# vectorch-ai/ScaleLLM

Hardware: AMD Instinct MI355X
Metric: decode tokens/s (Llama-3-8B-shaped step, bs=256, seq=4k; paged-attention HBM roofline + int4-GEMM TFLOP/s alongside) (higher is better)
Workload: dtype bf16 (int4 weights, fp32 accumulate)

## Files before the change

### include/slm_hip.h

```cpp
#ifndef SLM_HIP_H_
#define SLM_HIP_H_

#include <stddef.h>
#include <stdint.h>

#ifdef __cplusplus
extern "C" {
#endif

#define SLM_API __attribute__((visibility("default")))

typedef enum slm_status {
  SLM_OK = 0,
  SLM_ERR_INVALID_ARG = -1,
  SLM_ERR_UNSUPPORTED = -2,
  SLM_ERR_WORKSPACE = -3,
  SLM_ERR_LAUNCH = -4,
  SLM_ERR_ALIGNMENT = -5
} slm_status;

typedef enum slm_dtype {
  SLM_F16 = 0,
  SLM_BF16 = 1,
  SLM_F32 = 2
// ... 98 lines not shown
  const int32_t* perm;
  const void* bias;
  void* c;
  int64_t M, K, N;
  int64_t lda, ldc;
  int64_t group_size;
  int32_t dtype;
  int32_t flags;
  void* workspace;
  size_t workspace_bytes;
} slm_w4_gemm_args;

#define SLM_W4_DEFER_REDUCE 1
#define SLM_W4_SILU_MUL 2
#define SLM_W4_SHARES_CHIP 4

SLM_API size_t slm_w4a16_gemm_workspace_bytes(const slm_w4_gemm_args* a);
SLM_API int32_t slm_w4a16_gemm_deferred_splits(const slm_w4_gemm_args* a);
typedef enum slm_w4_kernel {
  SLM_W4_KERNEL_GEMV = 0,
  SLM_W4_KERNEL_KS = 1,
  SLM_W4_KERNEL_SMALL = 2,
  SLM_W4_KERNEL_GENERAL = 3,
  SLM_W4_KERNEL_M128 = 4,
  SLM_W4_KERNEL_WS = 5,
  SLM_W4_KERNEL_XL = 6,
  SLM_W4_KERNEL_XL_SK = 7
} slm_w4_kernel;
typedef struct slm_w4_plan_info {
  int32_t kernel;
  int32_t row_tiles;
  int32_t n_mblocks, n_nblocks, split_k, chunks_per_split;
  int32_t variant[4];
  uint64_t lds_bytes;
  uint64_t part_bytes, aperm_bytes;
} slm_w4_plan_info;
SLM_API int slm_w4a16_gemm_plan(const slm_w4_gemm_args* a, slm_w4_plan_info* out);
SLM_API int slm_w4a16_gemm(const slm_w4_gemm_args* a, void* stream);

typedef struct slm_w4_norm_prologue {
  const void* x;
  const float* partials;
// ... 479 lines not shown
```

### scalellm_amd/_lib.py

```python
from __future__ import annotations

import ctypes as C
import os

_HERE = os.path.dirname(os.path.abspath(__file__))
LIB_PATH = os.path.join(_HERE, "csrc", "libslm_hip.so")

SLM_F16, SLM_BF16 = 0, 1
SLM_F32 = 2
SLM_SAMPLE_MAX_TOP = 20
SLM_REJECTION_MAX_K = 16
SLM_W4_GPTQ, SLM_W4_AWQ = 0, 1
SLM_W8_GPTQ, SLM_W8_AWQ = 2, 3
SLM_W4_PAIRED = 0x10


class SlmError(RuntimeError):
    pass


class AttnArgs(C.Structure):
    _fields_ = [
        ("out", C.c_void_p), ("query", C.c_void_p), ("key_cache", C.c_void_p),
        ("value_cache", C.c_void_p),
# ... 13 lines not shown

class W4GemmArgs(C.Structure):
    _fields_ = [
        ("a", C.c_void_p), ("wq", C.c_void_p), ("sz", C.c_void_p), ("perm", C.c_void_p),
        ("bias", C.c_void_p), ("c", C.c_void_p),
        ("M", C.c_int64), ("K", C.c_int64), ("N", C.c_int64),
        ("lda", C.c_int64), ("ldc", C.c_int64), ("group_size", C.c_int64),
        ("dtype", C.c_int32), ("flags", C.c_int32),
        ("workspace", C.c_void_p), ("workspace_bytes", C.c_size_t),
    ]


SLM_W4_DEFER_REDUCE = 1
SLM_W4_SILU_MUL = 2
SLM_W4_SHARES_CHIP = 4

W4_KERNELS = ("GEMV", "KS", "SMALL", "GENERAL", "M128", "WS", "XL", "XL_SK")


class W4PlanInfo(C.Structure):
    _fields_ = [
        ("kernel", C.c_int32), ("row_tiles", C.c_int32), ("n_mblocks", C.c_int32),
        ("n_nblocks", C.c_int32), ("split_k", C.c_int32), ("chunks_per_split", C.c_int32),
        ("variant", C.c_int32 * 4),
        ("lds_bytes", C.c_uint64), ("part_bytes", C.c_uint64), ("aperm_bytes", C.c_uint64),
    ]

    @property
    def kernel_name(self) -> str:
        return W4_KERNELS[self.kernel]


# ... 354 lines not shown
```

### scalellm_amd/cpp_host.py

```python
from __future__ import annotations

import importlib.util
import os

_shim = None


def load_shim():
    global _shim
    if _shim is None:
        from .build_shim import build
        path = build()
        spec = importlib.util.spec_from_file_location("_slm_shim", path)
        mod = importlib.util.module_from_spec(spec)
        spec.loader.exec_module(mod)
        _shim = mod
    return _shim


def cpp_params(params):
    shim = load_shim()
    q = shim.InputParameters()
    q.num_sequences = int(params.q_cu_seq_lens.numel() - 1)
    q.q_cu_seq_lens, q.kv_cu_seq_lens = params.q_cu_seq_lens, params.kv_cu_seq_lens
# ... 7 lines not shown
    shim = load_shim()
    q = shim.SamplingParameters()
    names = ["temperatures", "top_p", "top_k", "do_sample", "seeds"]
    if sp.unique_token_ids is not None:
        names += ["frequency_penalties", "presence_penalties", "repetition_penalties", "unique_token_ids",
                  "unique_token_counts", "unique_token_ids_lens"]
    for name in names:
        t = getattr(sp, name)
        if t is not None:
            setattr(q, name, t)
    q.logprobs, q.max_top_logprobs = bool(sp.logprobs), int(sp.max_top_logprobs)
    return q


def from_decode_step(step, block_size: int, max_tokens: int, fused: bool = True, lanes: int = -1,
                     lanes_chain: bool = True, rank: int = 0, world_size: int = 1, kv_step=None):
    from .decode import hf_state_dict
    shim = load_shim()
    s = step.shape
    if getattr(step, "dense", False):
        raise ValueError("the C++ host step is built for int4 checkpoints: it has no unquantised form")
    qa = step.layers[0]["qkv"].quant_args
    if qa.bits != 4 or qa.desc_act:
        raise ValueError("the C++ host step is built for 4-bit, non-act-order checkpoints")
    m = shim.LlamaForCausalLMHip(hidden=s.hidden, n_heads=s.n_heads, n_kv_heads=s.n_kv_heads, head_dim=s.head_dim,
                                 intermediate=s.intermediate, n_layers=s.n_layers, vocab=s.vocab,
                                 max_position=s.max_position, rope_theta=s.rope_theta, rms_eps=s.rms_eps,
                                 quant_method=qa.quant_method, bits=4, group_size=qa.group_size, desc_act=False,
                                 max_tokens=max_tokens, fused=fused, decode_lanes=lanes, lanes_chain=lanes_chain,
                                 device_index=step.device.index or 0, rank=rank, world_size=world_size)
    m.load_state_dict(hf_state_dict(step))
    m.verify_loaded_weights()
    m.set_kv_caches([(L["kv"].key_cache, L["kv"].value_cache) for L in (kv_step or step).layers], block_size)
    m.set_cos_sin_cache(step.attn.handler.cos_sin)
    m.reserve(max_tokens)
    return m
```

### scalellm_amd/csrc/capi.hip

```cpp
#include <atomic>
#include <mutex>
#include <stdlib.h>
#include <string.h>

#include "common.h"
#include "tuning.h"

namespace slm {

namespace {
const char* const kTuneNames[TUNE_COUNT] = {
    "SLM_ATTN_NW",          "SLM_ATTN_SPLITS",      "SLM_ATTN_HGW",     "SLM_ATTN_TILE",
    "SLM_ATTN_TILE_SPLITS", "SLM_ATTN_TILE_PF",     "SLM_ATTN_U",       "SLM_ATTN_NT",
    "SLM_ATTN_TILE_DECODE", "SLM_ATTN_BAL",         "SLM_ATTN_W",       "SLM_ATTN_PRIO",
    "SLM_W4_GEMV",          "SLM_W4_GEMV_KS",   "SLM_W4_SMALL",
    "SLM_W4_MT",            "SLM_W4_MT_WIDE",       "SLM_W4_NTW",           "SLM_W4_PC",        "SLM_W4_SPLITK",
    "SLM_W4_POST",
    "SLM_W4_KS",            "SLM_W4_KS_CW",         "SLM_W4_KS_NW",     "SLM_W4_KS_TPW",
    "SLM_W4_KS_MT2",
    "SLM_W4_M128",          "SLM_W4_M128_WD",       "SLM_W4_M128_SPLITS",   "SLM_W4_M128_KW",   "SLM_W4_SPLIT_TARGET",
    "SLM_W4_M128_CT",       "SLM_ATTN_TILE_KV2",    "SLM_W4_XL_MODEL",      "SLM_W4_M128_ADMA",
    "SLM_W4_XL_SK",
    "SLM_LINEAR_SPLITK",    "SLM_LINEAR_RT",        "SLM_LINEAR_NW",
};
std::atomic<int32_t> g_tune[TUNE_COUNT];
std::once_flag g_tune_once;

void tune_init() {
  for (int k = 0; k < TUNE_COUNT; ++k) {
    const char* v = getenv(kTuneNames[k]);
    g_tune[k].store((v && *v) ? (int32_t)atoi(v) : TUNE_UNSET, std::memory_order_relaxed);
  }
}
int tune_index(const char* name) {
  if (!name) return -1;
  for (int k = 0; k < TUNE_COUNT; ++k)
    if (strcmp(name, kTuneNames[k]) == 0) return k;
  return -1;
// ... 146 lines not shown
```

### scalellm_amd/csrc/shim/slm_llama_hip.cpp

```cpp
#include "slm_llama_hip.h"

#include <ATen/hip/HIPEvent.h>
#include <ATen/hip/impl/HIPGuardImplMasqueradingAsCUDA.h>
#include <ATen/hip/impl/HIPStreamMasqueradingAsCUDA.h>
#include <c10/hip/HIPGraphsC10Utils.h>

#include <cmath>

#include "slm_hip.h"
#include "slm_rejection_sampler_hip.h"

namespace slm {
namespace {

using Stream = c10::hip::HIPStreamMasqueradingAsCUDA;

int dt(const torch::Tensor& t) { return t.scalar_type() == torch::kBFloat16 ? SLM_BF16 : SLM_F16; }
void* cur(const torch::Tensor& t) {
  return c10::hip::getCurrentHIPStreamMasqueradingAsCUDA(t.device().index()).stream();
}
void ok(int rc, const char* what) {
  TORCH_CHECK(rc == SLM_OK, what, " failed: ", slm_status_string(rc), " (", rc, ")",
              rc == SLM_ERR_LAUNCH ? slm_last_hip_error() : "");
}
// ... 370 lines not shown
void LlamaForCausalLMHip::run_two_lanes(Lane& l0, Lane& l1, std::vector<KVCache>& kv) {
  const auto dev = options_.device().index();
  const Stream main = c10::hip::getCurrentHIPStreamMasqueradingAsCUDA(dev);
  if (!side_stream_.has_value()) {
    TORCH_CHECK(!capturing(), "LlamaForCausalLMHip: call reserve() before capturing a two-lane step");
    side_stream_ = c10::hip::getStreamFromPoolMasqueradingAsCUDA(false, dev);
  }
  const Stream side = *side_stream_;
  std::vector<std::unique_ptr<at::cuda::CUDAEvent>> events;
  auto record = [&](const Stream& s) {
    events.push_back(std::make_unique<at::cuda::CUDAEvent>());
    events.back()->record(s);
    return events.back().get();
  };
  record(main)->block(side);
  struct ChipFlag { int& f; explicit ChipFlag(int& x) : f(x) { f = SLM_W4_SHARES_CHIP; } ~ChipFlag() { f = 0; } } chip(chip_flag_);
  Lane* lanes[2] = {&l0, &l1};
  const Stream streams[2] = {main, side};
  const size_t n = layers_.size();
  for (int i = 0; i < 2; ++i) {
    c10::hip::HIPStreamGuardMasqueradingAsCUDA g(streams[i]);
    pre_attn(*lanes[i], 0, kv);
  }
  at::cuda::CUDAEvent* prev = nullptr;
  for (size_t li = 0; li < n; ++li) {
    for (int i = 0; i < 2; ++i) {
      c10::hip::HIPStreamGuardMasqueradingAsCUDA g(streams[i]);
      if (prev != nullptr && opt_.lanes_chain) prev->block(streams[i]);
      attn(*lanes[i], li, kv, 1);
      prev = record(streams[i]);
      attn(*lanes[i], li, kv, 2);
// ... 156 lines not shown
```

### scalellm_amd/csrc/shim/slm_llama_hip.h

```cpp
#pragma once
#include <torch/torch.h>

#include <ATen/hip/impl/HIPStreamMasqueradingAsCUDA.h>

#include <memory>
#include <optional>
#include <string>
#include <vector>

#include "slm_attn_handler_hip.h"
#include "slm_qlinear_hip.h"
#include "slm_sampling_hip.h"
#include "slm_torch_shim.h"

namespace slm {

struct LlamaArgs {
  int64_t hidden_size = 4096;
  int64_t n_heads = 32;
  int64_t n_kv_heads = 8;
  int64_t head_dim = 128;
  int64_t intermediate_size = 14336;
  int64_t n_layers = 32;
  int64_t vocab_size = 128256;
  int64_t max_position_embeddings = 8192;
  float rope_theta = 500000.0f;
  float rms_norm_eps = 1e-5f;
};

class LlamaForCausalLMHip {
 public:
  struct Options {
    int64_t max_tokens = 256;
    bool fused = true;
    int64_t decode_lanes = -1;
    bool lanes_chain = true;
  };

  LlamaForCausalLMHip(const LlamaArgs& args, const QuantArgs& quant_args, const ParallelArgs& parallel_args,
                      const torch::TensorOptions& options, const Options& opt,
                      std::shared_ptr<FusedAllReduce> fused_allreduce = nullptr,
                      std::shared_ptr<FusedAllReduce> fused_allreduce_lane1 = nullptr);

  void load_state_dict(const StateDict& state_dict);
  void verify_loaded_weights() const;

  void reserve(int64_t n_tokens);

  torch::Tensor forward(const torch::Tensor& tokens, const torch::Tensor& positions,
                        std::vector<KVCache>& kv_caches, const InputParameters& input_params);
  torch::Tensor logits(const torch::Tensor& hidden_states, const torch::Tensor& selected_idxes);
// ... 76 lines not shown
```

### scalellm_amd/csrc/shim/slm_shim_pybind.cpp

```cpp
#include <ATen/hip/impl/HIPGuardImplMasqueradingAsCUDA.h>
#include <ATen/hip/impl/HIPStreamMasqueradingAsCUDA.h>
#include <torch/extension.h>

#include <algorithm>
#include <thread>

#include "slm_attn_handler_hip.h"
#include "slm_llama_hip.h"
#include "slm_mla_hip.h"
#include "slm_moe_hip.h"
#include "slm_permute_hip.h"
#include "slm_fp8_linear_hip.h"
#include "slm_linear_hip.h"
#include "slm_qlinear_hip.h"
#include "slm_rejection_sampler_hip.h"
#include "slm_sampling_hip.h"
#include "slm_torch_shim.h"

namespace py = pybind11;

PYBIND11_MODULE(_slm_shim, m) {
  m.doc() = "libtorch shim over libslm_hip (reference C++ operator signatures)";
  m.def("paged_kv_varlen_mha",
        [](torch::Tensor out, const torch::Tensor& query, const torch::Tensor& key_cache,
// ... 376 lines not shown
          auto v = value.view({T, n_kv_heads, head_dim});
          std::tie(q, k) = h.apply_pos_emb(q, k, positions);
          h.append_kv_cache(kv_cache, k, v, params);
        });
  struct PyLlama {
    std::unique_ptr<slm::ProcessGroup> pg;
    std::unique_ptr<slm::LlamaForCausalLMHip> model;
    std::vector<slm::KVCache> kv;
  };
  py::class_<PyLlama>(m, "LlamaForCausalLMHip")
      .def(py::init([make_args](int64_t hidden, int64_t n_heads, int64_t n_kv_heads, int64_t head_dim,
                                int64_t intermediate, int64_t n_layers, int64_t vocab, int64_t max_position,
                                double rope_theta, double rms_eps, const std::string& quant_method, int64_t bits,
                                int64_t group_size, bool desc_act, int64_t max_tokens, bool fused,
                                int64_t decode_lanes, bool lanes_chain, torch::ScalarType dtype, int device_index,
                                int rank, int world_size) {
             slm::LlamaArgs a;
             a.hidden_size = hidden; a.n_heads = n_heads; a.n_kv_heads = n_kv_heads; a.head_dim = head_dim;
             a.intermediate_size = intermediate; a.n_layers = n_layers; a.vocab_size = vocab;
             a.max_position_embeddings = max_position; a.rope_theta = static_cast<float>(rope_theta);
             a.rms_norm_eps = static_cast<float>(rms_eps);
             slm::LlamaForCausalLMHip::Options o;
             o.max_tokens = max_tokens; o.fused = fused; o.decode_lanes = decode_lanes; o.lanes_chain = lanes_chain;
             const bool awq = quant_method == "awq";
             auto p = std::make_unique<PyLlama>();
             const torch::Device dev(torch::kCUDA, device_index);
             if (world_size > 1) p->pg = std::make_unique<slm::LocalShardProcessGroup>(rank, world_size, dev);
             p->model = std::make_unique<slm::LlamaForCausalLMHip>(
                 a, make_args(quant_method, bits, group_size, desc_act, false, awq),
                 slm::ParallelArgs(rank, world_size, p->pg.get()), torch::dtype(dtype).device(dev), o);
             return p;
           }),
           py::arg("hidden"), py::arg("n_heads"), py::arg("n_kv_heads"), py::arg("head_dim"), py::arg("intermediate"),
           py::arg("n_layers"), py::arg("vocab"), py::arg("max_position"), py::arg("rope_theta"), py::arg("rms_eps"),
           py::arg("quant_method"), py::arg("bits"), py::arg("group_size"), py::arg("desc_act"), py::arg("max_tokens"),
           py::arg("fused") = true, py::arg("decode_lanes") = -1, py::arg("lanes_chain") = true,
           py::arg("dtype") = torch::kBFloat16, py::arg("device_index") = 0, py::arg("rank") = 0,
           py::arg("world_size") = 1)
      .def("n_local_heads", [](PyLlama& self) { return self.model->n_local_heads(); })
      .def("n_local_kv_heads", [](PyLlama& self) { return self.model->n_local_kv_heads(); })
      .def("load_state_dict",
           [](PyLlama& self, std::unordered_map<std::string, torch::Tensor> sd) {
             self.model->load_state_dict(slm::StateDict(std::move(sd)));
           })
      .def("verify_loaded_weights", [](PyLlama& self) { self.model->verify_loaded_weights(); })
      .def("set_kv_caches",
           [](PyLlama& self, const std::vector<std::pair<torch::Tensor, torch::Tensor>>& caches, int64_t block_size) {
             self.kv.clear();
             for (const auto& kvp : caches) self.kv.emplace_back(kvp.first, kvp.second, block_size);
           })
      .def("set_cos_sin_cache", [](PyLlama& self, const torch::Tensor& t) { self.model->handler().set_cos_sin_cache(t); })
      .def("reserve", [](PyLlama& self, int64_t n_tokens) { self.model->reserve(n_tokens); })
      .def("decode_step",
// ... 146 lines not shown
```

### scalellm_amd/csrc/tuning.h

```cpp
#pragma once
#include <stdint.h>

namespace slm {

enum TuneKey : int {
  TUNE_ATTN_NW = 0,
  TUNE_ATTN_SPLITS,
  TUNE_ATTN_HGW,
  TUNE_ATTN_TILE,
  TUNE_ATTN_TILE_SPLITS,
  TUNE_ATTN_TILE_PF,
  TUNE_ATTN_U,
  TUNE_ATTN_NT,
  TUNE_ATTN_TILE_DECODE,
  TUNE_ATTN_BAL,
  TUNE_ATTN_W,
  TUNE_ATTN_PRIO,
  TUNE_W4_GEMV,
  TUNE_W4_GEMV_KS,
  TUNE_W4_SMALL,
  TUNE_W4_MT,
  TUNE_W4_MT_WIDE,
  TUNE_W4_NTW,
  TUNE_W4_PC,
// ... 5 lines not shown
  TUNE_W4_KS_TPW,
  TUNE_W4_KS_MT2,
  TUNE_W4_M128,
  TUNE_W4_M128_WD,
  TUNE_W4_M128_SPLITS,
  TUNE_W4_M128_KW,
  TUNE_W4_SPLIT_TARGET,
  TUNE_W4_M128_CT,
  TUNE_ATTN_TILE_KV2,
  TUNE_W4_XL_MODEL,
  TUNE_W4_M128_ADMA,
  TUNE_W4_XL_SK,
  TUNE_LINEAR_SPLITK,
  TUNE_LINEAR_RT,
  TUNE_LINEAR_NW,
  TUNE_COUNT
};

constexpr int32_t TUNE_UNSET = INT32_MIN;

int tune_get(TuneKey k, int dflt);
bool tune_is_set(TuneKey k);

}
```

### scalellm_amd/csrc/w4.hip

```cpp
#include "w4_plan.h"
#include "tuning.h"

namespace slm {

__device__ __forceinline__ int awq_pos(int col_in_word) {
  return (col_in_word >> 1) + 4 * (col_in_word & 1);
}

__device__ __forceinline__ int64_t paired_src_col(int format, int64_t n_packed, int64_t N) {
  if (!(format & SLM_W4_PAIRED)) return n_packed;
  return (n_packed >> 6) * 32 + (n_packed & 31) + ((n_packed & 32) ? N / 2 : 0);
}

__global__ void __launch_bounds__(256) w4_prepack_weight_kernel(
    int format, const uint32_t* __restrict__ qweight, const int* __restrict__ perm, int64_t K,
    int64_t N, uint32_t* __restrict__ wq) {
  const int64_t widx = (int64_t)blockIdx.x * blockDim.x + threadIdx.x;
  if (widx >= N * K / 8) return;
  const int j = (int)(widx & 3);
  const int lane = (int)((widx >> 2) & 63);
  const int64_t tile = widx >> 8;
  const int64_t nt = tile % (N / 32), kt = tile / (N / 32);
  const int64_t n = paired_src_col(format, nt * 32 + (lane & 31), N);
  const int64_t kb = kt * 64 + j * 16 + (lane >> 5) * 8;
// ... 220 lines not shown
    kp.norm_eps = np->eps; kp.norm_res_in = np->residual_in; kp.norm_res_out = np->residual_out;
    kp.norm_weight = np->weight; kp.norm_out = np->normed_out;
  }
  if (a->perm) {
    uint16_t* ap = reinterpret_cast<uint16_t*>(reinterpret_cast<char*>(a->workspace) + pl.part_bytes);
    const unsigned gx = (unsigned)((a->K + 255) / 256);
    hipLaunchKernelGGL(w4_permute_cols_kernel, dim3(gx > 64 ? 64 : gx, (unsigned)a->M), dim3(256), 0,
                       st, reinterpret_cast<const uint16_t*>(a->a), a->perm, a->M, a->K, a->lda, ap);
    rc = hip_check_launch();
    if (rc != SLM_OK) return rc;
    kp.a = ap; kp.lda = a->K;
  }
  kp.wq = reinterpret_cast<const uint32_t*>(a->wq);
  kp.sz = reinterpret_cast<const uint32_t*>(a->sz);
  kp.bias = a->bias; kp.c = a->c;
  kp.part = pl.split_k > 1 ? reinterpret_cast<float*>(a->workspace) : nullptr;
  kp.M = a->M; kp.K = a->K; kp.N = a->N; kp.ldc = a->ldc;
  kp.gs_shift = (a->group_size == a->K) ? 30 : ilog2(a->group_size);
  kp.n_chunks = (int)(a->K / W4_KC);
  kp.split_k = pl.split_k; kp.chunks_per_split = pl.chunks_per_split;
  kp.n_mblocks = pl.n_mblocks; kp.n_nblocks = pl.n_nblocks;
  kp.silu = silu ? 1 : 0;
  kp.ks_tpw = pl.ks.tpw;
  kp.ks_groups = (int)(a->K / a->group_size);
  kp.sk_per = pl.xl_sk.sk_per; kp.sk_sync = nullptr; kp.sk_part = nullptr;
  switch (pl.kernel) {
    case W4Kernel::GEMV: launch_gemv(kp, a->dtype, pl, st); break;
    case W4Kernel::KS: launch_gemm_ks(kp, a->dtype, pl, st); break;
    case W4Kernel::SMALL: launch_gemm_small(kp, a->dtype, pl, st); break;
    case W4Kernel::GENERAL: launch_gemm_general(kp, a->dtype, pl, st); break;
    case W4Kernel::M128: launch_gemm_m128(kp, a->dtype, pl, st); break;
    case W4Kernel::WS: launch_gemm_ws(kp, a->dtype, pl, st); break;
    case W4Kernel::XL: launch_gemm_xl(kp, a->dtype, pl, st); break;
    case W4Kernel::XL_SK:
      kp.sk_part = reinterpret_cast<float*>(a->workspace);
      kp.sk_sync = reinterpret_cast<unsigned*>(reinterpret_cast<char*>(a->workspace) + W4_XL_SK_WGS * W4_XL_SK_SLOT_BYTES);
      if (hipMemsetAsync(kp.sk_sync, 0, W4_XL_SK_SYNC_BYTES, st) != hipSuccess) return hip_check_launch();
      launch_gemm_xl_sk(kp, a->dtype, pl, st);
      break;
  }
  rc = hip_check_launch();
  if (rc != SLM_OK) return rc;
  if (pl.split_k > 1 && !((a->flags & SLM_W4_DEFER_REDUCE) && !a->bias)) {
    dispatch_dtype(a->dtype, [&](auto t) {
      using T = decltype(t);
      if (silu) {
        const int64_t n4 = a->M * (a->N / 2) / 4;
        hipLaunchKernelGGL(w4_splitk_reduce_silu_kernel<T>, dim3((unsigned)((n4 + 255) / 256)), dim3(256), 0, st,
                           kp.part, a->bias, a->c, a->M, a->N, a->ldc, pl.split_k);
      } else {
        launch_splitk_reduce<T>(kp.part, a->bias, a->c, a->M, a->N, a->ldc, pl.split_k, st);
      }
    });
    rc = hip_check_launch();
  }
  return rc;
}

// ... 14 lines not shown
```

### scalellm_amd/csrc/w4_plan.h

```cpp
#pragma once
#include "w4_common.h"

namespace slm {

enum class W4Kernel : int {
  GEMV,
  KS,
  SMALL,
  GENERAL,
  M128,
  WS,
  XL,
  XL_SK,
};

struct GemmPlan {
  W4Kernel kernel;
  int ng;
  int split_k, chunks_per_split, n_mblocks, n_nblocks;
  size_t lds_bytes;
  size_t part_bytes, aperm_bytes;
  struct { int mt, ntw, pc, post; } general;
  struct { int mt, cw, nw, tpw; } ks;
  struct { int wd, kw, ct, adma; } m128;
  struct { int sk_per; } xl_sk;
  int n_blocks() const { return n_nblocks * n_mblocks * split_k; }
};

int plan_gemm(const slm_w4_gemm_args* a, GemmPlan* pl);

void launch_gemv(const GemmKParams& kp, int dtype, const GemmPlan& pl, hipStream_t st);
void launch_gemm_ks(const GemmKParams& kp, int dtype, const GemmPlan& pl, hipStream_t st);
void launch_gemm_small(const GemmKParams& kp, int dtype, const GemmPlan& pl, hipStream_t st);
void launch_gemm_general(const GemmKParams& kp, int dtype, const GemmPlan& pl, hipStream_t st);
void launch_gemm_m128(const GemmKParams& kp, int dtype, const GemmPlan& pl, hipStream_t st);
void launch_gemm_ws(const GemmKParams& kp, int dtype, const GemmPlan& pl, hipStream_t st);
void launch_gemm_xl(const GemmKParams& kp, int dtype, const GemmPlan& pl, hipStream_t st);
void launch_gemm_xl_sk(const GemmKParams& kp, int dtype, const GemmPlan& pl, hipStream_t st);

}
```

### scalellm_amd/csrc/w4_plan.hip

```cpp
#include "w4_plan.h"
#include "tuning.h"

namespace slm {

static int validate(const slm_w4_gemm_args* a) {
  if (!a) return SLM_ERR_INVALID_ARG;
  if (a->M < 0 || a->K <= 0 || a->N <= 0) return SLM_ERR_INVALID_ARG;
  if (a->dtype != SLM_F16 && a->dtype != SLM_BF16) return SLM_ERR_UNSUPPORTED;
  if (a->K % W4_KC || a->N % 32) return SLM_ERR_UNSUPPORTED;
  if (a->flags & ~(SLM_W4_DEFER_REDUCE | SLM_W4_SILU_MUL | SLM_W4_SHARES_CHIP)) return SLM_ERR_INVALID_ARG;
  if (a->flags & SLM_W4_SILU_MUL) {
    if (a->flags & SLM_W4_DEFER_REDUCE) return SLM_ERR_INVALID_ARG;
    if (a->N % 64) return SLM_ERR_UNSUPPORTED;
  }
  if (!w4_group_size_valid(a->group_size, a->K)) return SLM_ERR_UNSUPPORTED;
  return SLM_OK;
}

struct Shape {
  int n_chunks;
  int n_tiles;
  int64_t tiles4, tiles8, tiles16;
  bool silu;
  bool tables_fit_u32;
  bool a_fits_i31;
// ... 217 lines not shown
  if (ntw != 1 && ntw != 2) ntw = 1;
  if (mt >= 4) ntw = 1;
  const int pc = plan_tiles(a, s, mt, ntw, pl);
  if (mt >= 8) {
    pl->kernel = mt == 16 ? W4Kernel::XL : W4Kernel::WS;
    pl->lds_bytes = mt == 16 ? W4_XL_LDS_BYTES : W4_WS_LDS_BYTES;
    return true;
  }
  pl->kernel = W4Kernel::GENERAL;
  const int post = tune_get(TUNE_W4_POST, a->M <= 64 ? 1 : 0) != 0 && w4_post_fits(mt, ntw, pl->ng, pc);
  pl->general = {mt, ntw, pc, post};
  pl->lds_bytes = (size_t)2 * pc * 32 * mt * 256 + (post ? (size_t)2 * pc * pl->ng * 32 * mt * sizeof(float) : 0);
  return true;
}

int plan_gemm(const slm_w4_gemm_args* a, GemmPlan* pl) {
  const int rc = validate(a);
  if (rc != SLM_OK) return rc;
  const Shape s = shape_of(a);
  *pl = GemmPlan{};
  pl->ng = a->group_size == 32 ? 4 : a->group_size == 64 ? 2 : 1;
  const bool taken = plan_xl_sk(a, s, pl) || plan_gemv(a, s, pl) || plan_ks_one_tile(a, s, pl) ||
                     plan_ks_two_tiles(a, s, pl) || plan_small(a, s, pl) || plan_m128(a, s, pl) || plan_tiled(a, s, pl);
  (void)taken;
  pl->part_bytes = pl->split_k > 1 ? (size_t)pl->split_k * a->M * a->N * sizeof(float) : 0;
  if (pl->kernel == W4Kernel::XL_SK) pl->part_bytes = W4_XL_SK_WGS * W4_XL_SK_SLOT_BYTES + W4_XL_SK_SYNC_BYTES;
  pl->aperm_bytes = a->perm ? (((size_t)a->M * a->K * 2 + 255) & ~(size_t)255) : 0;
  return SLM_OK;
}

}

using namespace slm;

extern "C" {

SLM_API size_t slm_w4a16_gemm_workspace_bytes(const slm_w4_gemm_args* a) {
  GemmPlan pl;
  return plan_gemm(a, &pl) == SLM_OK ? pl.part_bytes + pl.aperm_bytes : 0;
}

SLM_API int32_t slm_w4a16_gemm_deferred_splits(const slm_w4_gemm_args* a) {
  GemmPlan pl;
  return plan_gemm(a, &pl) == SLM_OK && (a->flags & SLM_W4_DEFER_REDUCE) && !a->bias && pl.split_k > 1 ? pl.split_k : 0;
}

SLM_API int32_t slm_w4a16_gemv_norm_supported(const slm_w4_gemm_args* a) {
  GemmPlan pl;
  return plan_gemm(a, &pl) == SLM_OK && pl.kernel == W4Kernel::GEMV && !a->perm &&
         gemv_supported(a->M, a->K, a->group_size, true);
}

SLM_API int slm_w4a16_gemm_plan(const slm_w4_gemm_args* a, slm_w4_plan_info* out) {
  GemmPlan pl;
  if (!out) return SLM_ERR_INVALID_ARG;
  const int rc = plan_gemm(a, &pl);
  if (rc != SLM_OK) return rc;
  *out = slm_w4_plan_info{};
  out->kernel = (int32_t)pl.kernel;
// ... 2 lines not shown
  out->lds_bytes = pl.lds_bytes; out->part_bytes = pl.part_bytes; out->aperm_bytes = pl.aperm_bytes;
  auto variant = [&](int v0, int v1, int v2, int v3) {
    out->variant[0] = v0; out->variant[1] = v1; out->variant[2] = v2; out->variant[3] = v3;
  };
  switch (pl.kernel) {
    case W4Kernel::GEMV: out->row_tiles = 0; break;
    case W4Kernel::SMALL: out->row_tiles = 1; break;
    case W4Kernel::KS: out->row_tiles = pl.ks.mt; variant(pl.ks.mt, pl.ks.cw, pl.ks.nw, pl.ks.tpw); break;
    case W4Kernel::GENERAL:
      out->row_tiles = pl.general.mt;
      variant(pl.general.mt, pl.general.ntw, pl.general.pc, pl.general.post);
      break;
    case W4Kernel::M128: out->row_tiles = 4; variant(pl.m128.wd, pl.m128.kw, pl.m128.ct, pl.m128.adma); break;
    case W4Kernel::WS: case W4Kernel::XL: out->row_tiles = 8; break;
    case W4Kernel::XL_SK: out->row_tiles = 8; variant(pl.xl_sk.sk_per, 0, 0, 0); break;
  }
  return SLM_OK;
}

}
```

### scalellm_amd/decode.py

```python
from __future__ import annotations

import contextlib
import dataclasses
import os

from dataclasses import dataclass
from typing import List, Optional

import torch

from . import kernels
from .layers import (Attention, ColumnParallelFp8Linear, ColumnParallelLinear, ColumnParallelQLinear, HipAttnHandler,
                     InputParameters, KVCache, uniform_kv_hint, QuantArgs, RowParallelFp8Linear, RowParallelLinear,
                     RowParallelQLinear)
from .model_parallel import ParallelArgs


@dataclass
class LlamaShape:
    hidden: int = 4096
    n_heads: int = 32
    n_kv_heads: int = 8
    head_dim: int = 128
    intermediate: int = 14336
# ... 98 lines not shown
        dense = quant_method in ("none", "fp8")
        self.dense, self.weight_bits = dense, 8 if self.fp8 else 16 if dense else 4
        fuse_silu = fuse_silu and (shape.intermediate // pa.world_size) % 32 == 0
        self.ckpt = [] if keep_checkpoint else None
        if isinstance(custom_allreduce, (list, tuple)):
            self.custom_ars = [a for a in custom_allreduce if a is not None]
        else:
            self.custom_ars = [custom_allreduce] if custom_allreduce is not None else []
        self.custom_ar = self.custom_ars[0] if self.custom_ars else None
        self.shape, self.pa, self.dtype, self.device = shape, pa, dtype, torch.device(device)
        self.defer_splitk = os.environ.get("SLM_DEFER_SPLITK", "1") != "0"
        self.fold_norm = os.environ.get("SLM_FOLD_NORM", "1") != "0" and not dense
        _lm = os.environ.get("SLM_DECODE_LANES", "auto")
        self.lanes_min = (0 if dense else -1) if _lm == "auto" else int(_lm)
        self.lanes_chain = os.environ.get("SLM_DECODE_LANES_CHAIN", "1") != "0"
        self._side_stream = None
        self._lane_bufs = {}
        self._sample_bufs = None
        self.last_lanes = 1
        self._pinned_lanes = None
        tp = pa.world_size
        assert shape.n_heads % tp == 0 and shape.intermediate % tp == 0 and shape.hidden % tp == 0
        self.n_heads = shape.n_heads // tp
        self.n_kv_heads = max(shape.n_kv_heads // tp, 1)
        self.block_size = block_size
        D, H = shape.head_dim, shape.hidden
        gen = torch.Generator(device=self.device).manual_seed(seed * 1000 + 17)
        desc_act = desc_act and quant_method == "gptq"
        qa = QuantArgs(quant_method=quant_method, bits=bits, group_size=group_size,
                       zero_point=(quant_method == "awq"), desc_act=desc_act)
# ... 376 lines not shown
    def _run_two_lanes(self, l0, l1) -> None:
        main = torch.cuda.current_stream()
        if self._side_stream is None:
            self._side_stream = torch.cuda.Stream(device=self.device)
        side = self._side_stream
        l0.stream, l1.stream = main, side
        fork = torch.cuda.Event()
        fork.record(main)
        side.wait_event(fork)

        def on(ln):
            st = contextlib.ExitStack()
            st.enter_context(torch.cuda.stream(ln.stream))
            st.enter_context(kernels.workspace_lane(ln.idx))
            st.enter_context(kernels.shared_chip())
            return st
        n = len(self.layers)
        for ln in (l0, l1):
            with on(ln):
                self._first_norm(ln)
                self._pre_attn(ln, 0)
        prev = None
        for li in range(n):
            for ln in (l0, l1):
                with on(ln):
                    if prev is not None and self.lanes_chain:
                        ln.stream.wait_event(prev)
                    self._attn(ln, li, phase=1)
                    prev = torch.cuda.Event()
                    prev.record(ln.stream)
# ... 249 lines not shown
```

### scalellm_amd/kernels.py

```python
from __future__ import annotations

import contextlib
import threading
import ctypes as C
from typing import Optional

import torch

from . import _lib
from ._lib import SLM_BF16, SLM_F16, AttnArgs, SlmError, W4GemmArgs, check


def _dtype_code(t: torch.Tensor) -> int:
    if t.dtype == torch.bfloat16:
        return SLM_BF16
    if t.dtype == torch.float16:
        return SLM_F16
    raise SlmError(f"unsupported dtype {t.dtype}: fp16 / bf16 only")


def _require_gpu(*tensors: torch.Tensor) -> None:
    for t in tensors:
        if t is not None and not t.is_cuda:
            raise SlmError("scalellm_amd kernels need GPU tensors (no CPU fallback)")
# ... 54 lines not shown
        yield
    finally:
        _lane_tls.lane = prev


@contextlib.contextmanager
def shared_chip(on: bool = True):
    prev = getattr(_lane_tls, "shared", False)
    _lane_tls.shared = bool(on)
    try:
        yield
    finally:
        _lane_tls.shared = prev


def _chip_flag() -> int:
    return _lib.SLM_W4_SHARES_CHIP if getattr(_lane_tls, "shared", False) else 0


def _grow(table, nbytes: int, dev: torch.device, what: str) -> torch.Tensor:
    key = _dev_key(dev)
    ws = table.get(key)
    if ws is None or ws.numel() < nbytes:
        if torch.cuda.is_current_stream_capturing():
            kw = "sampling_nbytes" if table is _sampling_ws else "rejection_nbytes" if table is _rejection_ws else \
                "deferred_nbytes" if table is _deferred_ws or table is _deferred_ws_b else "nbytes"
            raise SlmError(f"{what} must be reserved before graph capture "
                           f"(need {nbytes} bytes): call reserve_workspace({kw}=...) first")
        size = max(int(nbytes), 1 << 20, 2 * ws.numel() if ws is not None else 0)
        if ws is not None:
            _retired.append(ws)
        ws = torch.empty(size, dtype=torch.uint8, device=dev)
# ... 422 lines not shown
    if n_tokens <= 0 or packed.perm is not None or dtype != packed.dtype:
        return False
    g = W4GemmArgs()
    g.a, g.wq, g.sz = None, packed.wq.data_ptr(), packed.sz.data_ptr()
    g.perm, g.bias, g.c = None, None, None
    g.M, g.K, g.N = n_tokens, packed.K, packed.N
    g.lda, g.ldc = packed.K, packed.N // 2 if silu_mul else packed.N
    g.group_size = packed.group_size
    g.dtype = SLM_BF16 if dtype == torch.bfloat16 else SLM_F16
    g.flags = _lib.SLM_W4_SILU_MUL if silu_mul else (_lib.SLM_W4_DEFER_REDUCE if defer_reduce else 0)
    g.workspace, g.workspace_bytes = None, 0
    return bool(_lib.lib().slm_w4a16_gemv_norm_supported(C.byref(g)))


def _set_gemm_flags(g: W4GemmArgs, defer_reduce: bool, silu_mul: bool) -> int:
    chip = _chip_flag()
    g.flags = chip
    if silu_mul:
        g.flags = _lib.SLM_W4_SILU_MUL | chip
    deferred = 0
    if defer_reduce:
        g.flags = _lib.SLM_W4_DEFER_REDUCE | chip
        deferred = _lib.lib().slm_w4a16_gemm_deferred_splits(C.byref(g))
        if not deferred:
            g.flags = chip
    return deferred


def w4_plan(a: torch.Tensor, packed: PackedW4, c: torch.Tensor, bias: Optional[torch.Tensor] = None,
            defer_reduce: bool = False, silu_mul: bool = False) -> "_lib.W4PlanInfo":
    g = _gemm_args(a, packed, c, bias, silu_mul)
# ... 1200 lines not shown
```

Before: 10660.

## Add fold kernel that reduces split-K partials in LDS within one workgroup

Adds a FOLD int4 GEMM kernel that runs the split-K slices as separate waves of one workgroup and sums their partial tiles through LDS. This replaces the separate partial-sum workspace pass and reduction kernel for small-M split-K GENERAL plans. It is enabled by default on decode lanes that share the chip. The change adds a block-level barrier loop and larger LDS use per workgroup, which may lower occupancy.

```diff
diff --git a/include/slm_hip.h b/include/slm_hip.h
--- a/include/slm_hip.h
+++ b/include/slm_hip.h
@@ -136,6 +136,7 @@
 #define SLM_W4_DEFER_REDUCE 1
 #define SLM_W4_SILU_MUL 2
 #define SLM_W4_SHARES_CHIP 4
+#define SLM_W4_FOLD_SPLITS 16
 
 SLM_API size_t slm_w4a16_gemm_workspace_bytes(const slm_w4_gemm_args* a);
 SLM_API int32_t slm_w4a16_gemm_deferred_splits(const slm_w4_gemm_args* a);
@@ -147,7 +148,8 @@
   SLM_W4_KERNEL_M128 = 4,
   SLM_W4_KERNEL_WS = 5,
   SLM_W4_KERNEL_XL = 6,
-  SLM_W4_KERNEL_XL_SK = 7
+  SLM_W4_KERNEL_XL_SK = 7,
+  SLM_W4_KERNEL_FOLD = 8
 } slm_w4_kernel;
 typedef struct slm_w4_plan_info {
   int32_t kernel;
diff --git a/scalellm_amd/_lib.py b/scalellm_amd/_lib.py
--- a/scalellm_amd/_lib.py
+++ b/scalellm_amd/_lib.py
@@ -51,8 +51,9 @@
 SLM_W4_DEFER_REDUCE = 1
 SLM_W4_SILU_MUL = 2
 SLM_W4_SHARES_CHIP = 4
-
-W4_KERNELS = ("GEMV", "KS", "SMALL", "GENERAL", "M128", "WS", "XL", "XL_SK")
+SLM_W4_FOLD_SPLITS = 16
+
+W4_KERNELS = ("GEMV", "KS", "SMALL", "GENERAL", "M128", "WS", "XL", "XL_SK", "FOLD")
 
 
 class W4PlanInfo(C.Structure):
diff --git a/scalellm_amd/cpp_host.py b/scalellm_amd/cpp_host.py
--- a/scalellm_amd/cpp_host.py
+++ b/scalellm_amd/cpp_host.py
@@ -2,6 +2,7 @@
 
 import importlib.util
 import os
+from typing import Optional
 
 _shim = None
 
@@ -45,7 +46,10 @@
 
 
 def from_decode_step(step, block_size: int, max_tokens: int, fused: bool = True, lanes: int = -1,
-                     lanes_chain: bool = True, rank: int = 0, world_size: int = 1, kv_step=None):
+                     lanes_chain: bool = True, rank: int = 0, world_size: int = 1, kv_step=None,
+                     lanes_fold: Optional[bool] = None):
+    if lanes_fold is None:
+        lanes_fold = bool(getattr(step, "lanes_fold", True))
     from .decode import hf_state_dict
     shim = load_shim()
     s = step.shape
@@ -59,7 +63,8 @@
                                  max_position=s.max_position, rope_theta=s.rope_theta, rms_eps=s.rms_eps,
                                  quant_method=qa.quant_method, bits=4, group_size=qa.group_size, desc_act=False,
                                  max_tokens=max_tokens, fused=fused, decode_lanes=lanes, lanes_chain=lanes_chain,
-                                 device_index=step.device.index or 0, rank=rank, world_size=world_size)
+                                 device_index=step.device.index or 0, rank=rank, world_size=world_size,
+                                 lanes_fold=lanes_fold)
     m.load_state_dict(hf_state_dict(step))
     m.verify_loaded_weights()
     m.set_kv_caches([(L["kv"].key_cache, L["kv"].value_cache) for L in (kv_step or step).layers], block_size)
diff --git a/scalellm_amd/csrc/capi.hip b/scalellm_amd/csrc/capi.hip
--- a/scalellm_amd/csrc/capi.hip
+++ b/scalellm_amd/csrc/capi.hip
@@ -22,6 +22,7 @@
     "SLM_W4_M128_CT",       "SLM_ATTN_TILE_KV2",    "SLM_W4_XL_MODEL",      "SLM_W4_M128_ADMA",
     "SLM_W4_XL_SK",
     "SLM_LINEAR_SPLITK",    "SLM_LINEAR_RT",        "SLM_LINEAR_NW",
+    "SLM_W4_FOLD",
 };
 std::atomic<int32_t> g_tune[TUNE_COUNT];
 std::once_flag g_tune_once;
diff --git a/scalellm_amd/csrc/shim/slm_llama_hip.cpp b/scalellm_amd/csrc/shim/slm_llama_hip.cpp
--- a/scalellm_amd/csrc/shim/slm_llama_hip.cpp
+++ b/scalellm_amd/csrc/shim/slm_llama_hip.cpp
@@ -408,7 +408,8 @@
     return events.back().get();
   };
   record(main)->block(side);
-  struct ChipFlag { int& f; explicit ChipFlag(int& x) : f(x) { f = SLM_W4_SHARES_CHIP; } ~ChipFlag() { f = 0; } } chip(chip_flag_);
+  struct ChipFlag { int& f; ChipFlag(int& x, int v) : f(x) { f = v; } ~ChipFlag() { f = 0; } } chip(
+      chip_flag_, SLM_W4_SHARES_CHIP | (opt_.lanes_fold ? SLM_W4_FOLD_SPLITS : 0));
   Lane* lanes[2] = {&l0, &l1};
   const Stream streams[2] = {main, side};
   const size_t n = layers_.size();
diff --git a/scalellm_amd/csrc/shim/slm_llama_hip.h b/scalellm_amd/csrc/shim/slm_llama_hip.h
--- a/scalellm_amd/csrc/shim/slm_llama_hip.h
+++ b/scalellm_amd/csrc/shim/slm_llama_hip.h
@@ -35,6 +35,7 @@
     bool fused = true;
     int64_t decode_lanes = -1;
     bool lanes_chain = true;
+    bool lanes_fold = true;
   };
 
   LlamaForCausalLMHip(const LlamaArgs& args, const QuantArgs& quant_args, const ParallelArgs& parallel_args,
diff --git a/scalellm_amd/csrc/shim/slm_shim_pybind.cpp b/scalellm_amd/csrc/shim/slm_shim_pybind.cpp
--- a/scalellm_amd/csrc/shim/slm_shim_pybind.cpp
+++ b/scalellm_amd/csrc/shim/slm_shim_pybind.cpp
@@ -414,7 +414,7 @@
                                 double rope_theta, double rms_eps, const std::string& quant_method, int64_t bits,
                                 int64_t group_size, bool desc_act, int64_t max_tokens, bool fused,
                                 int64_t decode_lanes, bool lanes_chain, torch::ScalarType dtype, int device_index,
-                                int rank, int world_size) {
+                                int rank, int world_size, bool lanes_fold) {
              slm::LlamaArgs a;
              a.hidden_size = hidden; a.n_heads = n_heads; a.n_kv_heads = n_kv_heads; a.head_dim = head_dim;
              a.intermediate_size = intermediate; a.n_layers = n_layers; a.vocab_size = vocab;
@@ -422,6 +422,7 @@
              a.rms_norm_eps = static_cast<float>(rms_eps);
              slm::LlamaForCausalLMHip::Options o;
              o.max_tokens = max_tokens; o.fused = fused; o.decode_lanes = decode_lanes; o.lanes_chain = lanes_chain;
+             o.lanes_fold = lanes_fold;
              const bool awq = quant_method == "awq";
              auto p = std::make_unique<PyLlama>();
              const torch::Device dev(torch::kCUDA, device_index);
@@ -436,7 +437,7 @@
            py::arg("quant_method"), py::arg("bits"), py::arg("group_size"), py::arg("desc_act"), py::arg("max_tokens"),
            py::arg("fused") = true, py::arg("decode_lanes") = -1, py::arg("lanes_chain") = true,
            py::arg("dtype") = torch::kBFloat16, py::arg("device_index") = 0, py::arg("rank") = 0,
-           py::arg("world_size") = 1)
+           py::arg("world_size") = 1, py::arg("lanes_fold") = true)
       .def("n_local_heads", [](PyLlama& self) { return self.model->n_local_heads(); })
       .def("n_local_kv_heads", [](PyLlama& self) { return self.model->n_local_kv_heads(); })
       .def("load_state_dict",
diff --git a/scalellm_amd/csrc/tuning.h b/scalellm_amd/csrc/tuning.h
--- a/scalellm_amd/csrc/tuning.h
+++ b/scalellm_amd/csrc/tuning.h
@@ -43,6 +43,7 @@
   TUNE_LINEAR_SPLITK,
   TUNE_LINEAR_RT,
   TUNE_LINEAR_NW,
+  TUNE_W4_FOLD,
   TUNE_COUNT
 };
 
diff --git a/scalellm_amd/csrc/w4.hip b/scalellm_amd/csrc/w4.hip
--- a/scalellm_amd/csrc/w4.hip
+++ b/scalellm_amd/csrc/w4.hip
@@ -258,7 +258,8 @@
   kp.wq = reinterpret_cast<const uint32_t*>(a->wq);
   kp.sz = reinterpret_cast<const uint32_t*>(a->sz);
   kp.bias = a->bias; kp.c = a->c;
-  kp.part = pl.split_k > 1 ? reinterpret_cast<float*>(a->workspace) : nullptr;
+  const bool fold = pl.kernel == W4Kernel::FOLD;
+  kp.part = (fold ? pl.part_bytes > 0 : pl.split_k > 1) ? reinterpret_cast<float*>(a->workspace) : nullptr;
   kp.M = a->M; kp.K = a->K; kp.N = a->N; kp.ldc = a->ldc;
   kp.gs_shift = (a->group_size == a->K) ? 30 : ilog2(a->group_size);
   kp.n_chunks = (int)(a->K / W4_KC);
@@ -282,10 +283,11 @@
       if (hipMemsetAsync(kp.sk_sync, 0, W4_XL_SK_SYNC_BYTES, st) != hipSuccess) return hip_check_launch();
       launch_gemm_xl_sk(kp, a->dtype, pl, st);
       break;
+    case W4Kernel::FOLD: launch_gemm_fold(kp, a->dtype, pl, st); break;
   }
   rc = hip_check_launch();
   if (rc != SLM_OK) return rc;
-  if (pl.split_k > 1 && !((a->flags & SLM_W4_DEFER_REDUCE) && !a->bias)) {
+  if (pl.split_k > 1 && !fold && !((a->flags & SLM_W4_DEFER_REDUCE) && !a->bias)) {
     dispatch_dtype(a->dtype, [&](auto t) {
       using T = decltype(t);
       if (silu) {
diff --git a/scalellm_amd/csrc/w4_fold.hip b/scalellm_amd/csrc/w4_fold.hip
--- /dev/null
+++ b/scalellm_amd/csrc/w4_fold.hip
@@ -0,0 +1,173 @@
+#include "w4_plan.h"
+#include "w4_epilogue.h"
+
+namespace slm {
+
+constexpr int W4_FOLD_PIECE_BYTES = 32 * 128;
+
+template <typename T, int NG>
+__global__ void __launch_bounds__(512, 4) w4a16_fold_kernel(const GemmKParams p) {
+  extern __shared__ __attribute__((aligned(16))) char smem[];
+  typedef typename Mfma<T>::frag frag_t;
+  constexpr int MTW = 2;
+  constexpr int PIECES = 2 * MTW;
+  constexpr int D = 2;
+  static_assert(PIECES % D == 0, "ring slots must stay compile-time per chunk");
+
+  const int tid = threadIdx.x;
+  const int lane = tid & 63;
+  const int wave = __builtin_amdgcn_readfirstlane(tid >> 6);
+  const int s = p.split_k;
+  const int rg = (int)(blockDim.x >> 6) / s;
+  const int ks = wave % s, grp = wave / s;
+  const int64_t ntile = blockIdx.x;
+  const int64_t n_tiles = p.N / 32;
+  const int c0 = ks * p.chunks_per_split;
+  const int c1 = min(p.n_chunks, c0 + p.chunks_per_split);
+  const int64_t g0 = (int64_t)blockIdx.y * rg;
+  const int64_t r0 = (g0 + grp) * (32 * MTW);
+  char* stage = smem + wave * W4_FOLD_PIECE_BYTES;
+
+  const __amdgpu_buffer_rsrc_t a_rs = w4_rsrc(p.a, (uint32_t)(((p.M - 1) * p.lda + p.K) * 2));
+  const __amdgpu_buffer_rsrc_t w_rs = w4_rsrc(p.wq, (uint32_t)((uint64_t)p.K * p.N / 2));
+  const __amdgpu_buffer_rsrc_t sz_rs = w4_rsrc(p.sz, (uint32_t)((uint64_t)p.ks_groups * p.N * 4));
+  const uint32_t row_bytes = (uint32_t)p.lda * 2u;
+
+  const uint32_t a_voff = (uint32_t)(lane >> 3) * row_bytes + (uint32_t)(lane & 7) * 16u;
+  auto a_load = [&](int c, int h, int m, u32x4 (&dst)[4]) {
+#pragma unroll
+    for (int i = 0; i < 4; ++i) {
+      const uint32_t off = (uint32_t)(r0 + m * 32 + 8 * i) * row_bytes + (uint32_t)c * 256u + (uint32_t)h * 128u;
+      dst[i] = __builtin_bit_cast(u32x4, __builtin_amdgcn_raw_buffer_load_b128(a_rs, (int)(a_voff + off), 0, 0));
+    }
+  };
+  auto a_store = [&](const u32x4 (&src)[4]) {
+#pragma unroll
+    for (int i = 0; i < 4; ++i) {
+      const int row = (lane >> 3) + 8 * i, slot = lane & 7;
+      *reinterpret_cast<u32x4*>(stage + row * 128 + ((slot ^ ((row >> 1) & 7)) << 4)) = src[i];
+    }
+  };
+
+  const uint32_t w_voff = (uint32_t)lane * 16u;
+  const uint32_t kt_stride = (uint32_t)n_tiles * 1024u;
+  auto w_load = [&](int c, u32x4 (&dst)[2]) {
+#pragma unroll
+    for (int h = 0; h < 2; ++h)
+      dst[h] = __builtin_bit_cast(u32x4, __builtin_amdgcn_raw_buffer_load_b128(
+                                             w_rs, (int)w_voff, (int)(((uint32_t)c * 2u + h) * kt_stride + (uint32_t)ntile * 1024u), 0));
+  };
+  const uint32_t sz_voff = (uint32_t)(lane & 31) * 4u;
+  const int cpg_shift = w4_cpg_shift(p.gs_shift);
+  auto sz_load = [&](int c, uint32_t (&dst)[NG]) {
+#pragma unroll
+    for (int g = 0; g < NG; ++g) {
+      const uint32_t grp_i = NG > 1 ? (uint32_t)c * NG + g : ((uint32_t)c >> cpg_shift);
+      dst[g] = (uint32_t)__builtin_amdgcn_raw_buffer_load_b32(sz_rs, (int)sz_voff,
+                                                              (int)(grp_i * (uint32_t)p.N * 4u + (uint32_t)ntile * 128u), 0);
+    }
+  };
+
+  f32x16 acc[MTW];
+#pragma unroll
+  for (int m = 0; m < MTW; ++m)
+#pragma unroll
+    for (int r = 0; r < 16; ++r) acc[m][r] = 0.f;
+
+  u32x4 wcur[2], wnxt[2];
+  uint32_t zcur[NG], znxt[NG];
+  u32x4 ring[D][4];
+  w_load(c0, wcur);
+  sz_load(c0, zcur);
+#pragma unroll
+  for (int q = 0; q < D; ++q) a_load(c0, q / MTW, q % MTW, ring[q]);
+
+  const int mrow = lane & 31, kh = lane >> 5;
+  for (int c = c0; c < c1; ++c) {
+    const int cn = c + 1 < c1 ? c + 1 : c;
+    w_load(cn, wnxt);
+    sz_load(cn, znxt);
+#pragma unroll
+    for (int h = 0; h < 2; ++h) {
+      frag_t bf[4];
+#pragma unroll
+      for (int j = 0; j < 4; ++j) {
+        const int w8 = h * 4 + j;
+        const uint32_t word = j == 0 ? wcur[h].x : j == 1 ? wcur[h].y : j == 2 ? wcur[h].z : wcur[h].w;
+        uint32_t o[4];
+        const W4Dq<T> dq(zcur[w8 * NG / 8]);
+        dq.word(word, o);
+        const u32x4 packed = {o[0], o[1], o[2], o[3]};
+        bf[j] = __builtin_bit_cast(frag_t, packed);
+      }
+#pragma unroll
+      for (int m = 0; m < MTW; ++m) {
+        const int q = h * MTW + m;
+        a_store(ring[q % D]);
+        const int qn = q + D;
+        if (qn < PIECES) a_load(c, qn / MTW, qn % MTW, ring[q % D]);
+        else a_load(cn, (qn - PIECES) / MTW, (qn - PIECES) % MTW, ring[q % D]);
+#pragma unroll
+        for (int j = 0; j < 4; ++j) {
+          const int slot = j * 2 + kh;
+          const u32x4 av = *reinterpret_cast<const u32x4*>(stage + mrow * 128 + ((slot ^ ((mrow >> 1) & 7)) << 4));
+          acc[m] = Mfma<T>::run(__builtin_bit_cast(frag_t, av), bf[j], acc[m]);
+        }
+      }
+    }
+#pragma unroll
+    for (int h = 0; h < 2; ++h) wcur[h] = wnxt[h];
+#pragma unroll
+    for (int g = 0; g < NG; ++g) zcur[g] = znxt[g];
+  }
+
+  float* fold = reinterpret_cast<float*>(smem);
+  const int64_t col0 = ntile * 32;
+  for (int g = 0; g < rg; ++g) {
+#pragma unroll
+    for (int m = 0; m < MTW; ++m) {
+      const int64_t prow = (g0 + g) * (32 * MTW) + m * 32;
+      if (prow >= p.M) continue;
+      __syncthreads();
+      if (grp == g) {
+#pragma unroll
+        for (int r = 0; r < 16; ++r) fold[ks * 1024 + r * 64 + lane] = acc[m][r];
+      }
+      __syncthreads();
+      for (int i = tid; i < 256; i += (int)blockDim.x) {
+        const int r = i >> 4, l0 = (i & 15) * 4;
+        const int64_t row = prow + cd_row(r, l0);
+        if (row >= p.M) continue;
+        f32x4 v = splitk_sum4(fold + r * 64 + l0, 1024, s);
+        const int64_t col = col0 + (l0 & 31);
+        if (p.part) {
+          *reinterpret_cast<f32x4*>(p.part + row * p.N + col) = v;
+        } else {
+          if (p.bias) {
+            const u32x2 b = *reinterpret_cast<const u32x2*>(reinterpret_cast<const uint16_t*>(p.bias) + col);
+            v.x += lo_f32<T>(b.x); v.y += hi_f32<T>(b.x);
+            v.z += lo_f32<T>(b.y); v.w += hi_f32<T>(b.y);
+          }
+          u32x2 o;
+          o.x = pack2<T>(v.x, v.y);
+          o.y = pack2<T>(v.z, v.w);
+          *reinterpret_cast<u32x2*>(reinterpret_cast<uint16_t*>(p.c) + row * p.ldc + col) = o;
+        }
+      }
+    }
+  }
+}
+
+void launch_gemm_fold(const GemmKParams& kp, int dtype, const GemmPlan& pl, hipStream_t st) {
+  const dim3 grid((unsigned)pl.n_nblocks, (unsigned)pl.n_mblocks), blk((unsigned)(64 * pl.split_k * pl.fold.rg));
+  dispatch_dtype(dtype, [&](auto t) {
+    using T = decltype(t);
+    switch (pl.ng) {
+      case 4: hipLaunchKernelGGL((w4a16_fold_kernel<T, 4>), grid, blk, pl.lds_bytes, st, kp); break;
+      case 2: hipLaunchKernelGGL((w4a16_fold_kernel<T, 2>), grid, blk, pl.lds_bytes, st, kp); break;
+      default: hipLaunchKernelGGL((w4a16_fold_kernel<T, 1>), grid, blk, pl.lds_bytes, st, kp); break;
+    }
+  });
+}
+
+}
diff --git a/scalellm_amd/csrc/w4_plan.h b/scalellm_amd/csrc/w4_plan.h
--- a/scalellm_amd/csrc/w4_plan.h
+++ b/scalellm_amd/csrc/w4_plan.h
@@ -12,6 +12,7 @@
   WS,
   XL,
   XL_SK,
+  FOLD,
 };
 
 struct GemmPlan {
@@ -24,6 +25,7 @@
   struct { int mt, cw, nw, tpw; } ks;
   struct { int wd, kw, ct, adma; } m128;
   struct { int sk_per; } xl_sk;
+  struct { int mtw, rg; } fold;
   int n_blocks() const { return n_nblocks * n_mblocks * split_k; }
 };
 
@@ -37,5 +39,6 @@
 void launch_gemm_ws(const GemmKParams& kp, int dtype, const GemmPlan& pl, hipStream_t st);
 void launch_gemm_xl(const GemmKParams& kp, int dtype, const GemmPlan& pl, hipStream_t st);
 void launch_gemm_xl_sk(const GemmKParams& kp, int dtype, const GemmPlan& pl, hipStream_t st);
+void launch_gemm_fold(const GemmKParams& kp, int dtype, const GemmPlan& pl, hipStream_t st);
 
 }
diff --git a/scalellm_amd/csrc/w4_plan.hip b/scalellm_amd/csrc/w4_plan.hip
--- a/scalellm_amd/csrc/w4_plan.hip
+++ b/scalellm_amd/csrc/w4_plan.hip
@@ -8,7 +8,8 @@
   if (a->M < 0 || a->K <= 0 || a->N <= 0) return SLM_ERR_INVALID_ARG;
   if (a->dtype != SLM_F16 && a->dtype != SLM_BF16) return SLM_ERR_UNSUPPORTED;
   if (a->K % W4_KC || a->N % 32) return SLM_ERR_UNSUPPORTED;
-  if (a->flags & ~(SLM_W4_DEFER_REDUCE | SLM_W4_SILU_MUL | SLM_W4_SHARES_CHIP)) return SLM_ERR_INVALID_ARG;
+  if (a->flags & ~(SLM_W4_DEFER_REDUCE | SLM_W4_SILU_MUL | SLM_W4_SHARES_CHIP | SLM_W4_FOLD_SPLITS))
+    return SLM_ERR_INVALID_ARG;
   if (a->flags & SLM_W4_SILU_MUL) {
     if (a->flags & SLM_W4_DEFER_REDUCE) return SLM_ERR_INVALID_ARG;
     if (a->N % 64) return SLM_ERR_UNSUPPORTED;
@@ -256,6 +257,22 @@
   return true;
 }
 
+static void plan_fold(const slm_w4_gemm_args* a, const Shape& s, GemmPlan* pl) {
+  if (!((a->flags & SLM_W4_FOLD_SPLITS) && tune_get(TUNE_W4_FOLD, 1) != 0 && pl->kernel == W4Kernel::GENERAL &&
+        pl->split_k > 1 && pl->split_k <= 8 && !pl->general.post && a->M <= 128 && !s.silu && s.tables_fit_u32 &&
+        a->lda * 256 < ((int64_t)1 << 31)))
+    return;
+  int groups = (int)((a->M + 63) / 64);
+  if (groups < 1) groups = 1;
+  const int rg = pl->split_k * groups <= 8 ? groups : 1;
+  pl->kernel = W4Kernel::FOLD;
+  pl->general = {0, 0, 0, 0};
+  pl->fold = {2, rg};
+  pl->n_mblocks = groups / rg;
+  pl->n_nblocks = s.n_tiles;
+  pl->lds_bytes = (size_t)pl->split_k * rg * 32 * 128;
+}
+
 int plan_gemm(const slm_w4_gemm_args* a, GemmPlan* pl) {
   const int rc = validate(a);
   if (rc != SLM_OK) return rc;
@@ -265,8 +282,11 @@
   const bool taken = plan_xl_sk(a, s, pl) || plan_gemv(a, s, pl) || plan_ks_one_tile(a, s, pl) ||
                      plan_ks_two_tiles(a, s, pl) || plan_small(a, s, pl) || plan_m128(a, s, pl) || plan_tiled(a, s, pl);
   (void)taken;
+  plan_fold(a, s, pl);
   pl->part_bytes = pl->split_k > 1 ? (size_t)pl->split_k * a->M * a->N * sizeof(float) : 0;
   if (pl->kernel == W4Kernel::XL_SK) pl->part_bytes = W4_XL_SK_WGS * W4_XL_SK_SLOT_BYTES + W4_XL_SK_SYNC_BYTES;
+  if (pl->kernel == W4Kernel::FOLD)
+    pl->part_bytes = (a->flags & SLM_W4_DEFER_REDUCE) && !a->bias ? (size_t)a->M * a->N * sizeof(float) : 0;
   pl->aperm_bytes = a->perm ? (((size_t)a->M * a->K * 2 + 255) & ~(size_t)255) : 0;
   return SLM_OK;
 }
@@ -284,7 +304,8 @@
 
 SLM_API int32_t slm_w4a16_gemm_deferred_splits(const slm_w4_gemm_args* a) {
   GemmPlan pl;
-  return plan_gemm(a, &pl) == SLM_OK && (a->flags & SLM_W4_DEFER_REDUCE) && !a->bias && pl.split_k > 1 ? pl.split_k : 0;
+  if (!(plan_gemm(a, &pl) == SLM_OK && (a->flags & SLM_W4_DEFER_REDUCE) && !a->bias && pl.split_k > 1)) return 0;
+  return pl.kernel == W4Kernel::FOLD ? 1 : pl.split_k;
 }
 
 SLM_API int32_t slm_w4a16_gemv_norm_supported(const slm_w4_gemm_args* a) {
@@ -317,6 +338,10 @@
     case W4Kernel::M128: out->row_tiles = 4; variant(pl.m128.wd, pl.m128.kw, pl.m128.ct, pl.m128.adma); break;
     case W4Kernel::WS: case W4Kernel::XL: out->row_tiles = 8; break;
     case W4Kernel::XL_SK: out->row_tiles = 8; variant(pl.xl_sk.sk_per, 0, 0, 0); break;
+    case W4Kernel::FOLD:
+      out->row_tiles = pl.fold.mtw * pl.fold.rg;
+      variant(pl.fold.mtw, pl.fold.rg, pl.split_k * pl.fold.rg, 0);
+      break;
   }
   return SLM_OK;
 }
diff --git a/scalellm_amd/decode.py b/scalellm_amd/decode.py
--- a/scalellm_amd/decode.py
+++ b/scalellm_amd/decode.py
@@ -136,6 +136,7 @@
         _lm = os.environ.get("SLM_DECODE_LANES", "auto")
         self.lanes_min = (0 if dense else -1) if _lm == "auto" else int(_lm)
         self.lanes_chain = os.environ.get("SLM_DECODE_LANES_CHAIN", "1") != "0"
+        self.lanes_fold = os.environ.get("SLM_DECODE_LANES_FOLD", "1") != "0"
         self._side_stream = None
         self._lane_bufs = {}
         self._sample_bufs = None
@@ -542,6 +543,7 @@
             st.enter_context(torch.cuda.stream(ln.stream))
             st.enter_context(kernels.workspace_lane(ln.idx))
             st.enter_context(kernels.shared_chip())
+            st.enter_context(kernels.fold_splits(self.lanes_fold))
             return st
         n = len(self.layers)
         for ln in (l0, l1):
diff --git a/scalellm_amd/kernels.py b/scalellm_amd/kernels.py
--- a/scalellm_amd/kernels.py
+++ b/scalellm_amd/kernels.py
@@ -92,8 +92,22 @@
         _lane_tls.shared = prev
 
 
+@contextlib.contextmanager
+def fold_splits(on: bool = True):
+    prev = getattr(_lane_tls, "fold", False)
+    _lane_tls.fold = bool(on)
+    try:
+        yield
+    finally:
+        _lane_tls.fold = prev
+
+
 def _chip_flag() -> int:
     return _lib.SLM_W4_SHARES_CHIP if getattr(_lane_tls, "shared", False) else 0
+
+
+def _w4_lane_flags() -> int:
+    return _chip_flag() | (_lib.SLM_W4_FOLD_SPLITS if getattr(_lane_tls, "fold", False) else 0)
 
 
 def _grow(table, nbytes: int, dev: torch.device, what: str) -> torch.Tensor:
@@ -546,7 +560,7 @@
 
 
 def _set_gemm_flags(g: W4GemmArgs, defer_reduce: bool, silu_mul: bool) -> int:
-    chip = _chip_flag()
+    chip = _w4_lane_flags()
     g.flags = chip
     if silu_mul:
         g.flags = _lib.SLM_W4_SILU_MUL | chip
```

After: 9763. 0.916x the previous value.
